# chrhansk/sleqp

Hardware: AMD Instinct MI355X
Metric: KKT factor+solve/sec (numeric refactor + 1 solve with device-controlled refinement, inputs resident in HBM) (higher is better)
Workload: dtype f64; 1 GPU; banded_n1e5_m5e4; n=100000, m=50000, N=150000, nnz_J=1000000, nnz_tril_K=1100000, nnz_L=11646539, nnz_L_stored=12226637, supernodes=569, etree_levels=10, refine_steps=1, hip_graphs=5, solves_per_factor=1, parallelism=single

## Files before the change

sleqp_amd/csrc/abi_options.inc:

```
enum OptionEffect {
  FX_NONE,
  FX_GRAPHS,
  FX_GRAPHS_IF_CHANGED,
  FX_PLANS,
  FX_PLANS_IF_CHANGED,
};
struct OptionRow {
  const char* name;
  const char* env;
  OptionEffect effect;
  int (*set)(hipfact_handle* h, double v);
  const char* doc;
};
#define OPT_STORE(field, conv)                 \
  [](hipfact_handle* h, double v) -> int {     \
    const auto x = (conv);                     \
    const bool changed = h->field != x;        \
    h->field = x;                              \
    return changed;                            \
  }
static const OptionRow kOptions[] = {
    {"refine_steps", "HIPFACT_REFINE", FX_GRAPHS,
     [](hipfact_handle* h, double v) -> int {
       h->refine_steps = std::max(0, (int)v);
// ... 146 lines not shown
    {"profile", nullptr, FX_NONE,
     [](hipfact_handle* h, double v) -> int {
       if (h->prof.on) prof_collect(h);
       if (v < 0)
         for (int c = 0; c < PC_COUNT; ++c) h->prof.ms[c] = 0, h->prof.max_ms[c] = 0, h->prof.cnt[c] = 0;
       h->prof.tagged.clear();
       h->prof.on = v > 0;
       return 1;
     },
     "event-time every kernel class; value < 0 resets the counters"},
    {"ordering", nullptr, FX_PLANS, OPT_STORE(prm.ordering, (int)v),
     "0 nested dissection + AMD leaves (default), 1 AMD on the whole graph, 2 natural"},
    {"max_children", nullptr, FX_PLANS, OPT_STORE(prm.max_children, (int)v),
     "relaxed amalgamation keeps fronts at this many children (default 4 = what the pull extend-add takes in one block)"},
    {"force_generic", nullptr, FX_PLANS, OPT_STORE(prm.force_generic, v != 0.0),
     "1: no saddle-point structure detection, static 1 x 1 pivots on K as given (symmetric positive definite input: the PSD shim)"},
    {"dense_mode", nullptr, FX_PLANS, OPT_STORE(prm.dense_mode, std::min(2, std::max(0, (int)v))),
     "1: late elimination inside the tree (default), 2: low-rank correction, 0: off"},
    {nullptr, "HIPFACT_DATAFLOW_RETRY", FX_NONE, OPT_STORE(df_retry_every, std::max(0, (int)v)), nullptr},
    {nullptr, "HIPFACT_CHECK_LAUNCHES", FX_NONE, OPT_STORE(check_launches, v != 0.0), nullptr},
    {nullptr, "HIPFACT_SOL_SPLIT", FX_NONE, OPT_STORE(sol_split, v != 0.0), nullptr},
    {nullptr, "HIPFACT_IDX64", FX_NONE, OPT_STORE(idx64, v != 0.0), nullptr},
    {nullptr, "HIPFACT_XCD_CLASSES", FX_NONE, OPT_STORE(xcd_classes, std::max(1, std::min(XCD_CLASSES_MAX, (int)v))), nullptr},
};
#undef OPT_STORE

static void options_from_environment(hipfact_handle* h) {
  for (const OptionRow& row : kOptions)
    if (const char* s = row.env ? getenv(row.env) : nullptr) (void)row.set(h, (double)atoi(s));
}

int hipfact_set_option(hipfact_handle* h, const char* name, double value) {
  if (!h || !name) return HIPFACT_EINVAL;
  {
    bool known = false;
    const int rc = multi_set_option(h, name, value, known);
    if (known) return rc;
  }
  {
    bool known = false;
    const int rc = condest_set_option(h, name, value, known);
    if (known) return rc;
  }
  for (const OptionRow& row : kOptions) {
    if (!row.name || strcmp(name, row.name)) continue;
    const int changed = row.set(h, value);
// ... 20 lines not shown
  };
  const Plan& P = h->plan;
  if (!strcmp(name, "perm")) return host_copy(P.perm);
  if (!strcmp(name, "sn_c0")) return host_copy(P.sn_c0);
  if (!strcmp(name, "sn_r")) return host_copy(P.sn_r);
  if (!strcmp(name, "sn_rowptr")) return host_copy(P.sn_rowptr);
  if (!strcmp(name, "sn_rows")) return host_copy(P.sn_rows);
  if (!strcmp(name, "sn_Loff")) return host_copy(P.sn_Loff);
  if (!strcmp(name, "late_cols")) return host_copy(P.late_cols);
  if (!strcmp(name, "sn_level")) return host_copy(P.sn_level);
  if (!strcmp(name, "dense_cols")) return host_copy(P.dense_cols);
  if (!strcmp(name, "cond_history")) return host_copy(h->cond_history);
  const DevBuf* b = nullptr;
  if (!strcmp(name, "L")) b = &h->d_L;
  else if (!strcmp(name, "U")) b = &h->d_U;
  else if (!strcmp(name, "SPf")) b = &h->d_SPf;
  else if (!strcmp(name, "sitems")) b = &h->d_sitems;
  else if (!strcmp(name, "y")) b = &h->d_y;
  else if (!strcmp(name, "xhat")) b = &h->d_xhat;
  else if (!strcmp(name, "ysol")) b = &h->d_ysol;
  else if (!strcmp(name, "uvec")) b = &h->d_uvec;
  else if (!strcmp(name, "dscale")) b = &h->d_dscale;
  else if (!strcmp(name, "Kval")) b = &h->d_Kval;
  else if (!strcmp(name, "mY")) b = &h->d_mY;
  if (!strcmp(name, "cond_d")) {
    const size_t N = (size_t)h->N_ext, off = (2 * COND_T + 3) * N * sizeof(double);
    if (!h->d_cblk.p || bytes > N * sizeof(double)) {
      h->error = "hipfact_debug_copy: unknown buffer or size";
      return HIPFACT_EINVAL;
    }
    HCHECK(h, hipStreamSynchronize(h->stream));
    HCHECK(h, hipMemcpy(out, h->d_cblk.as<char>() + off, bytes, hipMemcpyDeviceToHost));
    return HIPFACT_OK;
  }
  if (!b || !b->p || bytes > b->bytes) {
    h->error = "hipfact_debug_copy: unknown buffer or size";
    return HIPFACT_EINVAL;
  }
  HCHECK(h, hipStreamSynchronize(h->stream));
  HCHECK(h, hipMemcpy(out, b->p, bytes, hipMemcpyDeviceToHost));
  return HIPFACT_OK;
}

int hipfact_debug_place_rows(int m, const int* Ar_ptr, long long fill_bytes, int classes, long long* bounds, int* classes_out,
                             int* grid_out, int* blocks) {
  if (m < 0 || (m > 0 && !Ar_ptr) || fill_bytes < 0 || classes < 1 || classes > XCD_CLASSES_MAX || !bounds || !classes_out ||
// ... 182 lines not shown
  INFO("multi_passes", h->multi_passes) INFO("multi_single_cols", h->multi_single_cols) INFO("multi_failed_col", h->multi_failed_col)
  INFO("multi_sliced_fronts", h->mitems_for < 0 ? 0 : h->n_mcut) INFO("multi_slice_items", h->mitems_for < 0 ? 0 : h->n_mslices) INFO("multi_slice_rows", h->multi_slice_rows)
  INFO("cond_estimates", h->cond_estimates) INFO("cond_blocks", h->cond_blocks) INFO("cond_last", h->cond_last) INFO("condition_estimate", h->condition_estimate)
  INFO("extra_solves", h->extra_solves) INFO("extra_passes", h->extra_passes) INFO("extra_last_status", h->extra_last_status)
  INFO("extra_multi_solves", h->extra_multi_solves) INFO("extra_multi_cols", h->extra_multi_cols) INFO("extra_multi_passes", h->extra_multi_passes)
  INFO("num_solve", h->num_solve) INFO("num_refined", h->solve_cad.num_refined) INFO("refine_adaptive", h->refine_adaptive)
  INFO("num_passes", h->solve_cad.num_passes) INFO("last_omega", h->last_ctl.omega) INFO("last_iters", h->last_ctl.iters)
  INFO("last_status", h->last_ctl.status) INFO("last_tol", h->last_ctl.tol) INFO("kappa_est", h->last_ctl.kappa)
  INFO("refine_inline", h->factor_cad.refine_inline) INFO("refine_tol", h->refine_tol) INFO("equilibrate", h->equilibrate)
  INFO("factor_top_level", h->ftop_level) INFO("factor_top_count", h->ftop_count) INFO("solve_timeouts", h->h_info.p ? h->h_info.as<int>()[INFO_TIMEOUT] : 0)
  INFO("top_level", 1 << 30)
  INFO("use_graph", h->use_graph) INFO("num_graphs", h->graphs.size()) INFO("max_r", P.max_r) INFO("max_w", P.max_w) INFO("refine_steps", h->refine_steps)
  INFO("schur_flops_max_level", h->schur_flops_max)
  INFO("chain_pairs", h->n_pairs)
  INFO("xupd_fused", h->xupd_fused ? 1 : 0)
  INFO("rhs_in_tree", h->last_rhs_in_tree) INFO("xupd_in_tree", h->last_xupd_in_tree) INFO("xupd_blocks_launched", h->last_xupd_blocks)
  INFO("solve_sliced_fronts", h->n_sliced) INFO("solve_resorted_levels", h->n_resorted) INFO("tree_solve", tree_solve(h))
  INFO("refine_check_every", h->refine_check_every) INFO("refine_check_interval", h->solve_cad.check_interval_now) INFO("num_checked", h->solve_cad.num_checked)
  INFO("device", h->device) INFO("nnzM", P.Mi.size()) INFO("nnzA", P.Ar_src.size())
  INFO("rows_total", P.sn_rows.size()) INFO("ent_fused", h->ent_fused) INFO("ent_split", h->ent_split)
  INFO("rows_fused", h->rows_fused) INFO("rows_split", h->rows_split)
  INFO("long_row_segments", h->n_rseg) INFO("row_scale_blocks", row_scale_in_sequence(h) ? h->rs_grid : 0)
  INFO("arena_fill_bytes", arena_fill_bytes(P))
  INFO("xcd_classes", h->xcd_classes) INFO("dealt_multi_item_fronts", h->dealt_multi) INFO("long_prod_segments", h->n_lprod)
  INFO("long_col_segments", h->n_cseg) INFO("idx32", h->idx32) INFO("prod_packed", h->prod_packed)
  INFO("active_bounds", h->maps_on ? h->n_bounds : 0)
  INFO("values_in_place",
       h->have_plan && (!h->from_jacobian || (virtual_current(h) && h->vj->identity))) INFO("inactive_rows", h->maps_on ? h->n_inactive : 0)
#undef INFO
  return HIPFACT_EINVAL;
}
```

sleqp_amd/csrc/kernel_types.h:

```cpp
#pragma once
#include <hip/hip_runtime.h>

#include "device_types.h"

namespace hipfact {

constexpr int FB = 256;
constexpr int MV_LONG = 4096;
constexpr int CL = 8;
constexpr int SB = 1024;
constexpr int DOT_BLOCKS = 128;
constexpr int RL = 16;
constexpr int ST = 1024;
constexpr int SPB = 512;
constexpr int ZT = 64;
constexpr int ZC = 32;
constexpr int ZS = 512;
constexpr int CG_BLOCKS = 2048;
constexpr int CG_CHUNK = 8;

constexpr int MR = 16;
constexpr int MB = 1024;

struct RefineCtl {
// ... 53 lines not shown
  double* __restrict__ segpart;
  unsigned int* __restrict__ segcnt;
};
struct RhsIn {
  const int* __restrict__ Ar_ptr;
  const int* __restrict__ Ar_col;
  const double* __restrict__ Ar_val;
  const int* __restrict__ perm;
  SaddleMaps M;
  const double* __restrict__ b;
};
struct XupdIn {
  int n;
  const int* __restrict__ Kp;
  const double* __restrict__ Ksc;
  const int* __restrict__ Kc_y;
  const int* __restrict__ perm;
  SaddleMaps M;
  const double* __restrict__ b;
  double* __restrict__ z;
  int acc;
  int nblocks;
  double* __restrict__ dot_out;
};
struct CgCtl {
  double rg, z_nrm_sq, rel_tol_sq, rad_sq, alpha, beta, tau;
  double ray_min, ray_max;
  int state;
  int stop, apply, it, max_iter, pad;
};
struct LzCtl {
  double tol, rad_sq, gamma0;
  double gam_prev, gam_cur;
  double del_cur;
  double piv, fsub;
  double rho, s_nrm_sq, sp, p_nrm_sq;
  int k;
  int stop;
  int state;
  int kmax;
};

}
```

sleqp_amd/csrc/kernels_saddle.inc:

```




__global__ __launch_bounds__(FB) void k_row_scale(int m, const int* __restrict__ Ar_ptr,
                                                  const int* __restrict__ Ar_col, const int* __restrict__ Ar_src,
                                                  const double* __restrict__ Kval, const int* __restrict__ vmap,
                                                  const int* __restrict__ dmask, const int* __restrict__ perm,
                                                  int late_my, int enable, double* __restrict__ dscale,
                                                  double* __restrict__ Ar_val, double* __restrict__ Ar_full,
                                                  double* __restrict__ Ksc, double* __restrict__ Kprod,
                                                  double* __restrict__ Kcopy, long long nnzK,
                                                  double2* __restrict__ zero,
                                                  long long nzero, int* __restrict__ info, int nrseg,
                                                  const LongSeg* __restrict__ rseg, DecideIn D, int decide,
                                                  ClassBounds RB) {
  const int nbw = gridDim.x, bid = blockIdx.x;
  if (bid == 0) {
    if (decide && D.ctl->pending) dev_refine_decide(D, 1);
    __syncthreads();
    if (threadIdx.x < INFO_BYTES / 4) info[threadIdx.x] = 0;
  }
  if (Kcopy)
    for (long long i = bid * (long long)FB + threadIdx.x; i < nnzK; i += (long long)nbw * FB) Kcopy[i] = Kval[i];
  const int sub = threadIdx.x % RL;
// ... 150 lines not shown
                                                   const int* __restrict__ perm, SaddleMaps M,
                                                   const double* __restrict__ b, double* __restrict__ t,
                                                   const int* __restrict__ skip) {
  if (skip && *skip) return;
  const RhsIn R{Ar_ptr, Ar_col, Ar_val, perm, M, b};
  const int sub = threadIdx.x % RL;
  const int rpb = FB / RL;
  for (int k = blockIdx.x * rpb + threadIdx.x / RL; k < m; k += gridDim.x * rpb) {
    const double s = rhs_row(R, k, sub);
    if (sub == 0 && R.Ar_ptr[k + 1] - R.Ar_ptr[k] <= LONG_ROW) t[k] = s;
  }
  if (M.nrseg > 0) {
    __shared__ double lsum[FB / 64];
    rhs_long_rows<FB>(R, blockIdx.x, gridDim.x, t, lsum);
  }
}

template <bool ACC>
__global__ __launch_bounds__(FB) void k_x_saddle(int n, int m, const int* __restrict__ Kp,
                                                 const double* __restrict__ Ksc, const int* __restrict__ Kc_y,
                                                 const int* __restrict__ perm, SaddleMaps M,
                                                 const double* __restrict__ yp, const double* __restrict__ b,
                                                 double* __restrict__ z, const int* __restrict__ skip,
                                                 int* __restrict__ epoch) {
  if (skip && *skip) return;
  if (epoch && blockIdx.x == 0 && threadIdx.x == 0) *epoch += 1;
  const int sub = threadIdx.x % CL;
  const int cpb = FB / CL;
  for (int j = blockIdx.x * cpb + threadIdx.x / CL; j < n; j += gridDim.x * cpb) {
    double s = 0.0;
    const int e1 = Kp[j + 1];
    if (e1 - Kp[j] - 1 > LONG_COL) continue;
    for (int e = Kp[j] + 1 + sub; e < e1; e += CL) s += Ksc[e] * yp[Kc_y[e]];
#pragma unroll
    for (int o = CL / 2; o > 0; o >>= 1) s += __shfl_down(s, o, CL);
    if (sub == 0) (void)x_col_write(M, j, s, b, z, ACC ? 1 : 0);
  }
  if (M.ncseg > 0) {
    __shared__ double lsum[FB / 64];
    (void)x_long_cols<false, FB>(M, blockIdx.x, gridDim.x, Kp, Ksc, Kc_y, yp, b, z, ACC ? 1 : 0, nullptr, lsum);
  }
  for (int k = blockIdx.x * FB + threadIdx.x; k < m; k += gridDim.x * FB) {
    const int i = ext_row(M, perm[k]);
    if (i >= 0) {
      const double v = yp[k] * M.dscale[k];
      if (ACC)
        z[i] += v;
      else
        z[i] = v;
    }
  }
}


__device__ __forceinline__ void resid_col_tail(const SaddleMaps& M, int j, double s, const double* __restrict__ b,
                                               const double* __restrict__ z, double* __restrict__ res, double& mr,
                                               double& mb, double& mz) {
  const double bj = b[j], zj = z[j];
  const int v = M.vmap ? M.vmap[j] : -1;
// ... 14 lines not shown
}
__device__ __forceinline__ void resid_row_tail(const SaddleMaps& M, int k, const int* __restrict__ perm, double s,
                                               const double* __restrict__ b, const double* __restrict__ z,
                                               double* __restrict__ res, double& mr, double& mb, double& mz) {
  const int i = ext_row(M, perm[k]);
  if (i >= 0) {
    const double d = M.dscale[k];
    const double bi = b[i] * d;
    const double ri = bi - s;
    res[i] = ri / d;
    mr = nanmax(mr, fabs(ri));
    mb = fmax(mb, fabs(bi));
    mz = fmax(mz, fabs(z[i] / d));
  }
}

__global__ __launch_bounds__(FB) void k_residual_saddle(int n, int m, const int* __restrict__ Kp,
                                                        const int* __restrict__ Ki, const double* __restrict__ Kval,
                                                        const int* __restrict__ Ar_ptr, const int* __restrict__ Ar_col,
                                                        const double* __restrict__ Ar_val,
                                                        const int* __restrict__ perm, SaddleMaps M,
                                                        const double* __restrict__ b, const double* __restrict__ z,
                                                        double* __restrict__ res, const RefineCtl* __restrict__ ctl,
                                                        double* __restrict__ partials, int first, int* __restrict__ defer) {
  if (ctl && !first && ctl->done) return;
  double mr = 0.0, mb = 0.0, mz = 0.0;
  __shared__ double lsum[FB / 64];
  const int nbx = (int)gridDim.x >> 1;
  if ((int)blockIdx.x < nbx) {
    const int sub = threadIdx.x % CL;
    const int cpb = FB / CL;
    const int iters = (n + nbx * cpb - 1) / (nbx * cpb);
    for (int it = 0; it < iters; ++it) {
      const int j = (it * nbx + blockIdx.x) * cpb + threadIdx.x / CL;
      double s = 0.0;
      bool mine = j < n;
      if (mine) {
        const int e1 = Kp[j + 1];
        if (e1 - Kp[j] - 1 > LONG_COL)
          mine = false;
        else
          for (int e = Kp[j] + sub; e < e1; e += CL) {
            const int i = Ki[e];
            const int zi = i < n ? i : ext_row(M, i - n);
            if (zi >= 0) s += Kval[e] * z[zi];
          }
      }
#pragma unroll
      for (int o = CL / 2; o > 0; o >>= 1) s += __shfl_down(s, o, CL);
      if (sub == 0 && mine) resid_col_tail(M, j, s, b, z, res, mr, mb, mz);
    }
    for (int q = blockIdx.x; q < M.ncseg; q += nbx) {
      const LongSeg sg = M.cseg[q];
      const int j = sg.id;
      double s = 0.0;
// ... 78 lines not shown
```

sleqp_amd/csrc/kernels_solve.hip:

```cpp
#include <hip/hip_runtime.h>

#include "device_types.h"
#include "kernel_types.h"

namespace hipfact {
#include "kernels_common.inc"
#include "kernels_residual_common.inc"
#include "kernels_solve_level.inc"
#include "kernels_solve_multi.inc"
#include "kernels_solve_tree.inc"
#include "kernels_saddle.inc"
#include "kernels_vector.inc"
}

#define DENSE_COLS_KERNELS
#include "dense_cols.inc"
#undef DENSE_COLS_KERNELS
#define KRYLOV_DEVICE_KERNELS
#include "krylov_device.inc"
#undef KRYLOV_DEVICE_KERNELS
#define KRYLOV_LSQR_KERNELS
#include "krylov_lsqr.inc"
#undef KRYLOV_LSQR_KERNELS

// ... 17 lines not shown
INST_CGH(64)
#undef INST_CGH
#define INST_LZ(L)                                                                                                  \
  template __global__ void k_lz_spmv_dot<L>(int, const LzCtl*, const int*, const int*, const double*, const int*,   \
                                            const int*, const double*, const double*, double*, double*);
INST_LZ(1)
INST_LZ(4)
INST_LZ(16)
INST_LZ(64)
#undef INST_LZ
#define INST_LSQR(L)                                                                                                  \
  template __global__ void k_lsqr_forward<L>(int, int, const int*, const int*, const double*, const double*,         \
                                             const int*, const int*, const double*, const double*, double, double,   \
                                             double*, double*);                                                      \
  template __global__ void k_lsqr_adjoint<L>(int, int, const int*, const int*, const double*, const double*,         \
                                             const int*, const int*, const double*, const double*, const double*,    \
                                             int, double*, double*);
INST_LSQR(1)
INST_LSQR(4)
INST_LSQR(16)
INST_LSQR(64)
#undef INST_LSQR
template __global__ void k_x_saddle<true>(int, int, const int*, const double*, const int*, const int*, SaddleMaps,
                                          const double*, const double*, double*, const int*, int*);
template __global__ void k_x_saddle<false>(int, int, const int*, const double*, const int*, const int*, SaddleMaps,
                                           const double*, const double*, double*, const int*, int*);
}
```

sleqp_amd/csrc/kernels_solve_tree.inc:

```

__device__ __forceinline__ void dev_refine_decide(const DecideIn& D, int first) {
  RefineCtl* __restrict__ ctl = D.ctl;
  RefineCtl* __restrict__ hctl = D.hctl;
  __shared__ double sh[3][16];
  const int tid = threadIdx.x, nthr = blockDim.x;
  double r = 0.0, bb = 0.0, zz = 0.0;
  for (int q = tid; q < D.nblk; q += nthr) {
    r = nanmax(r, D.partials[3 * q]);
    bb = nanmax(bb, D.partials[3 * q + 1]);
    zz = nanmax(zz, D.partials[3 * q + 2]);
  }
#pragma unroll
  for (int o = 32; o > 0; o >>= 1) {
    r = nanmax(r, __shfl_down(r, o, 64));
    bb = nanmax(bb, __shfl_down(bb, o, 64));
    zz = nanmax(zz, __shfl_down(zz, o, 64));
  }
  if ((tid & 63) == 0) {
    sh[0][tid >> 6] = r;
    sh[1][tid >> 6] = bb;
    sh[2][tid >> 6] = zz;
  }
  __syncthreads();
  if (tid == 0) {
// ... 512 lines not shown
                                              double* __restrict__ z, int acc) {
  const int v = M.vmap ? M.vmap[j] : -1;
  const double bj = b[j];
  if (v >= 0) {
    const double beta = b[v];
    const double mult = (bj - beta) - s;
    if (acc) {
      z[j] += beta;
      z[v] += mult;
    } else {
      z[j] = beta;
      z[v] = mult;
    }
    return bj * beta;
  }
  if (acc) {
    z[j] += bj - s;
    return 0.0;
  }
  const double zj = bj - s;
  z[j] = zj;
  return bj * zj;
}
template <bool POLL, int NT>
__device__ __forceinline__ double x_long_cols(const SaddleMaps& M, int bid, int nb, const int* __restrict__ Kp,
                                              const double* __restrict__ Ksc, const int* __restrict__ Kc_y,
                                              const double* __restrict__ ys, const double* __restrict__ b,
                                              double* __restrict__ z, int acc, int* __restrict__ info, double* lds) {
  double dsum = 0.0;
  for (int q = bid; q < M.ncseg; q += nb) {
    const LongSeg sg = M.cseg[q];
    double s = 0.0;
    for (int e = sg.begin + (int)threadIdx.x; e < sg.end; e += NT)
      s += Ksc[e] * (POLL ? poll_f64(ys + Kc_y[e], info) : ys[Kc_y[e]]);
    s = block_sum_fixed<NT>(s, lds);
    double tot;
    if (threadIdx.x == 0 && seg_arrive(s, sg.poff, sg.idx, sg.nseg, M.segpart, M.segcnt + sg.uid, tot))
      dsum += x_col_write(M, sg.id, tot, b, z, acc);
  }
  return dsum;
}
__device__ __forceinline__ void dev_x_update(const XupdIn& X, int xb, const double* __restrict__ ys, int m,
                                             int* __restrict__ info, double* lds) {
  constexpr int XL = 8, XE = 2, XP = 4;
  const int sub = threadIdx.x % XL;
  const int cpb = ST / XL;
  const int stride = X.nblocks * cpb;
  const SaddleMaps& M = X.M;
  const unsigned long long* __restrict__ yb = reinterpret_cast<const unsigned long long*>(ys);
  const int k0 = xb * ST + threadIdx.x, kstride = X.nblocks * ST;
  int yi = -1;
  double ysc = 0.0, dsum = 0.0;
  if (k0 < m) {
    yi = ext_row(M, X.perm[k0]);
    ysc = M.dscale[k0];
  }
  for (int jb = xb * cpb + threadIdx.x / XL; jb < X.n; jb += XP * stride) {
    double val[XP][XE];
    int idx[XP][XE], enext[XP], eend[XP];
    bool colok[XP];
#pragma unroll
    for (int p = 0; p < XP; ++p) {
      const int j = jb + p * stride;
      bool ok = j < X.n;
      int e0 = ok ? X.Kp[j] + 1 + sub : 0, e1 = ok ? X.Kp[j + 1] : 0;
      if (e1 - (e0 - sub) > LONG_COL) e1 = e0 = 0, ok = false;
      colok[p] = ok;
#pragma unroll
      for (int t = 0; t < XE; ++t) {
        const int e = e0 + XL * t;
        val[p][t] = (e < e1) ? X.Ksc[e] : 0.0;
        idx[p][t] = (e < e1) ? X.Kc_y[e] : -1;
      }
      enext[p] = e0 + XL * XE;
      eend[p] = e1;
    }
    unsigned long long bits[XP][XE];
#pragma unroll
    for (int p = 0; p < XP; ++p)
#pragma unroll
      for (int t = 0; t < XE; ++t)
        bits[p][t] = (idx[p][t] >= 0) ? __hip_atomic_load(yb + idx[p][t], __ATOMIC_RELAXED, __HIP_MEMORY_SCOPE_AGENT) : 0ull;
#pragma unroll
    for (int p = 0; p < XP; ++p) {
      const int j = jb + p * stride;
      double s = 0.0;
#pragma unroll
      for (int t = 0; t < XE; ++t)
        if (idx[p][t] >= 0) {
          const double yv = (bits[p][t] == SOLVE_SENT) ? poll_f64(ys + idx[p][t], info) : __longlong_as_double((long long)bits[p][t]);
          s += val[p][t] * yv;
        }
      for (int e = enext[p]; e < eend[p]; e += XL) s += X.Ksc[e] * poll_f64(ys + X.Kc_y[e], info);
#pragma unroll
      for (int o = XL / 2; o > 0; o >>= 1) s += __shfl_down(s, o, XL);
      if (sub == 0 && colok[p]) dsum += x_col_write(M, j, s, X.b, X.z, X.acc);
    }
  }
  if (M.ncseg > 0) {
    const double dl = x_long_cols<true, ST>(M, xb, X.nblocks, X.Kp, X.Ksc, X.Kc_y, ys, X.b, X.z, X.acc, info, lds);
    if (threadIdx.x == 0) dsum += dl;
    __syncthreads();
  }
  if (X.dot_out) {
    dsum = wave_sum(dsum);
    if ((threadIdx.x & 63) == 0) lds[threadIdx.x >> 6] = dsum;
    __syncthreads();
    if (threadIdx.x == 0) {
      double a = 0.0;
      for (int q = 0; q < ST / 64; ++q) a += lds[q];
      X.dot_out[xb] = a;
    }
  }
  for (int k = k0; k < m; k += kstride) {
    const int i = (k == k0) ? yi : ext_row(M, X.perm[k]);
    if (i >= 0) {
      const double v = poll_f64(ys + k, info) * ((k == k0) ? ysc : M.dscale[k]);
      if (X.acc)
        X.z[i] += v;
// ... 68 lines not shown
```

sleqp_amd/csrc/runtime_extra.inc:

```

struct ExtraRule {
  int nblk = 1, cap = 1;
  int k = 0;
  int applied = 0;
  int status = -1;
  double rho = 0.0, ferr = INFINITY, dz_rel = INFINITY;
  double dn_prev[2] = {0.0, 0.0};
};
static inline double extra_rel(double dn, double zn) { return dn == 0.0 ? 0.0 : dn / zn; }
static bool extra_rule_step(ExtraRule& R, const double* dn, const double* zn) {
  const double eps = std::ldexp(1.0, -53);
  ++R.k;
  bool finite = true;
  for (int q = 0; q < R.nblk; ++q) finite = finite && std::isfinite(dn[q]) && std::isfinite(zn[q]);
  if (!finite) {
    R.status = HIPFACT_EXTRA_NONFINITE;
    R.ferr = R.dz_rel = INFINITY;
    return false;
  }
  double ratio = 0.0;
  if (R.k >= 2) {
    for (int q = 0; q < R.nblk; ++q)
      if (R.dn_prev[q] > 0.0) ratio = std::max(ratio, dn[q] / R.dn_prev[q]);
    R.rho = std::max(R.rho, ratio);
// ... 15 lines not shown
    R.status = HIPFACT_EXTRA_PASS_LIMIT;
  return true;
}

static void residual_dd_async(hipfact_handle* h, const double* b, const double* z, double* res, double* partials) {
  const Plan& P = h->plan;
  if (P.saddle) {
    LAUNCH(PC_RESID, k_residual_saddle_dd, dim3(resid_blocks(P)), dim3(FB), 0, P.n, P.m, h->d_Kp.as<int>(),
           h->d_Ki.as<int>(), h->d_Kval.as<double>(), h->d_Ar_ptr.as<int>(), h->d_Ar_col.as<int>(),
           (masked_rows(h) ? h->d_Ar_full : h->d_Ar_val).as<double>(), h->d_perm.as<int>(), saddle_maps(h), b, z, res,
           partials);
  } else {
    LAUNCH(PC_RESID, k_residual_sym_dd, dim3(resid_blocks(P)), dim3(FB), 0, P.N, h->d_Kp.as<int>(), h->d_Ki.as<int>(),
           h->d_Kval.as<double>(), h->d_Tp.as<int>(), h->d_Ti.as<int>(), h->d_Tsrc.as<int>(), b, z, res, partials);
  }
}

static void residual_fp64_async(hipfact_handle* h, const double* b, const double* z, double* res) {
  const Plan& P = h->plan;
  if (P.saddle) {
    LAUNCH(PC_RESID, k_residual_saddle, dim3(resid_blocks(P)), dim3(FB), 0, P.n, P.m, h->d_Kp.as<int>(),
           h->d_Ki.as<int>(), h->d_Kval.as<double>(), h->d_Ar_ptr.as<int>(), h->d_Ar_col.as<int>(),
           (masked_rows(h) ? h->d_Ar_full : h->d_Ar_val).as<double>(), h->d_perm.as<int>(), saddle_maps(h), b, z, res,
           (const RefineCtl*)nullptr, (double*)nullptr, 1, (int*)nullptr);
  } else {
    LAUNCH(PC_RESID, k_residual_sym, dim3(resid_blocks(P)), dim3(FB), 0, P.N, h->d_Kp.as<int>(), h->d_Ki.as<int>(),
           h->d_Kval.as<double>(), h->d_Tp.as<int>(), h->d_Ti.as<int>(), h->d_Tsrc.as<int>(), b, z, res,
           (const RefineCtl*)nullptr, (double*)nullptr, 1, (int*)nullptr);
  }
}

static const int g_maxabs_cap = 256;

static int extra_workspace(hipfact_handle* h) {
  const size_t N = (size_t)h->N_ext;
  hipError_t e = h->d_xvec.ensure(std::max<size_t>(4 * N * sizeof(double), 16));
  if (e == hipSuccess) e = h->d_xctl.ensure(sizeof(RefineCtl));
  if (e == hipSuccess) e = h->d_xnorms.ensure((size_t)3 * g_resid_cap * sizeof(double));
  if (e == hipSuccess) e = h->d_xpart.ensure((size_t)4 * g_maxabs_cap * sizeof(double));
  if (e == hipSuccess && !h->h_xout.p) {
    e = h->h_xout.ensure(4 * sizeof(double) + sizeof(RefineCtl));
    if (e == hipSuccess) e = hipHostGetDevicePointer(&h->h_xout_dev, h->h_xout.p, 0);
  }
  if (e != hipSuccess) {
    (void)hipGetLastError();
    h->d_xvec.release();
    h->error = std::string("hipfact_solve_device_extra: workspace: ") + hipGetErrorString(e);
// ... 106 lines not shown
```

sleqp_amd/csrc/runtime_queue.inc:

```
struct TurnState {
  std::mutex mu;
  hipEvent_t last = nullptr;
  hipfact_handle* owner = nullptr;
  std::atomic<int> live{0};
};
static TurnState g_turn[16];
static hipfact_handle* g_trace_handles[8] = {nullptr};
struct Turn {
  hipfact_handle* h;
  bool counted = false, held = false;
  explicit Turn(hipfact_handle* h_) : h(h_) {
    if (h->capturing) return;
    counted = true;
    if (h->turn_depth++ > 0) return;
    TurnState& T = g_turn[h->device & 15];
    static const bool off = getenv("HIPFACT_NO_TURNS") != nullptr;
    if (off || T.live.load(std::memory_order_acquire) <= 1 || !h->ev_turn) return;
    T.mu.lock();
    held = true;
    if (T.last && T.owner != h) {
      (void)hipStreamWaitEvent(h->stream, T.last, 0);
      h->turn_waits++;
    }
  }
// ... 21 lines not shown
      break;
    }
}
static void turn_leave(hipfact_handle* h) {
  TurnState& T = g_turn[h->device & 15];
  std::lock_guard<std::mutex> g(T.mu);
  T.live.fetch_sub(1, std::memory_order_acq_rel);
  for (auto& g : g_trace_handles)
    if (g == h) g = nullptr;
  if (T.owner == h) {
    T.owner = nullptr;
    T.last = nullptr;
  }
}

static DecideIn decide_in(hipfact_handle* h, int col = -1);
static inline bool diag_inactive_needed(const hipfact_handle* h) {
  const Plan& P = h->plan;
  return P.saddle && P.m > 0 && ((h->maps_on && h->n_inactive > 0) || P.n_late > 0);
}
static inline bool row_scale_in_sequence(const hipfact_handle* h) {
  const Plan& P = h->plan;
  return P.saddle && P.n > 0 && P.m > 0;
}
static inline bool dataflow_factor(const hipfact_handle* h) { return h->debug_phases == 15 && !h->no_dataflow; }
static inline bool tree_solve(const hipfact_handle* h) { return h->fused_solve && !h->no_dataflow; }
static inline bool tree_delivers_verdict(const hipfact_handle* h) { return tree_solve(h) && h->plan.m > 0 && h->plan.saddle; }
static inline bool graph_route(const hipfact_handle* h) { return h->use_graph && !h->prof.on && h->debug_phases == 15; }
static inline const int* cmap_or_null(const hipfact_handle* h) { return (h->maps_on || h->plan.n_late > 0) ? h->d_cmap.as<int>() : nullptr; }
static inline bool masked_rows(const hipfact_handle* h) { return h->nd > 0 || h->plan.n_late > 0; }
static inline size_t arena_fill_bytes(const Plan& P) {
  return (size_t)P.L_size * sizeof(double) + (size_t)4 * P.nsuper * sizeof(int);
}
static inline int row_scale_grid(long long m, size_t fill_bytes) {
  const long long nz16 = (long long)((fill_bytes + 15) / 16);
  const int for_fill = (int)std::min<long long>(2048, std::max<long long>(1, nz16 / (FB * 8)));
  return std::max(nblocks(m * 16), for_fill);
}
static int place_rows(int m, const int* Ar_ptr, size_t fill_bytes, int classes, ClassBounds& cb) {
  return place_ranges((long long)m, FB / RL, Ar_ptr, LONG_ROW, classes, row_scale_grid(m, fill_bytes), (long long)((fill_bytes + 15) / 16), cb);
}
static void place_front_end(hipfact_handle* h) {
  const Plan& P = h->plan;
  h->rs_grid = place_rows(P.m, P.Ar_ptr.data(), arena_fill_bytes(P), h->xcd_classes, h->rs_place);
}
template <bool CH>
// ... 350 lines not shown
           h->d_info.as<int>(), skip, rhs ? *rhs : RhsIn{},
           decide_in(h), h->d_spart.as<double>(), X);
    return;
  }
  for (int l = 0; l < P.nlevels; ++l) {
    const LevelInfo& li = h->levels[l];
    LAUNCH(PC_FWD, k_fwd_level, dim3(li.count), dim3(SB), li.lds_fwd, h->d_sn.as<SnDesc>(),
           h->d_level_sn.as<int>() + li.begin, h->d_L.as<double>(), h->d_rel.as<int>(), h->d_child.as<int>(),
           h->d_y.as<double>(), h->d_uvec.as<double>(), skip);
  }
  for (int l = P.nlevels - 1; l >= 0; --l) {
    const LevelInfo& li = h->levels[l];
    LAUNCH(PC_BWD, k_bwd_level, dim3(li.count), dim3(SB), li.lds_bwd, h->d_sn.as<SnDesc>(),
           h->d_level_sn.as<int>() + li.begin, h->d_L.as<double>(), h->d_rows.as<int>(), h->d_y.as<double>(), skip);
  }
}

static void launch_rhs_saddle(hipfact_handle* h, const SaddleMaps& M, const double* b, const int* skip, double* y = nullptr) {
  const Plan& P = h->plan;
  LAUNCH(PC_RHS, k_rhs_saddle, dim3(nblocks((long long)P.m * 16)), dim3(FB), 0, P.m, h->d_Ar_ptr.as<int>(),
         h->d_Ar_col.as<int>(), h->d_Ar_val.as<double>(), h->d_perm.as<int>(), M, b, y ? y : h->d_y.as<double>(), skip);
}
static void launch_x_saddle(hipfact_handle* h, const SaddleMaps& M, const double* b, double* z, bool acc, const int* skip,
                            int* epoch, const double* y = nullptr) {
  const Plan& P = h->plan;
  auto go = [&](auto ACC) {
    LAUNCH(PC_XUPD, k_x_saddle<decltype(ACC)::value>, dim3(nblocks((long long)P.n * 8)), dim3(FB), 0, P.n, P.m, h->d_Kp.as<int>(),
           h->d_Ksc.as<double>(), h->d_Kc_y.as<int>(), h->d_perm.as<int>(), M, y ? y : h->d_y.as<double>(), b, z, skip, epoch);
  };
  acc ? go(std::true_type()) : go(std::false_type());
}

static void launch_rhs_perm(hipfact_handle* h, const double* b, const int* skip, double* y = nullptr) {
  const Plan& P = h->plan;
  LAUNCH(PC_PERM, k_gather_skip, dim3(nblocks(P.m)), dim3(FB), 0, (long long)P.m, h->d_perm.as<int>(), b,
         y ? y : h->d_y.as<double>(), skip);
}
static void launch_x_perm(hipfact_handle* h, double* z, bool acc, const int* skip, int* epoch, const double* y = nullptr) {
  const Plan& P = h->plan;
  if (!y) y = h->d_y.as<double>();
  if (acc)
    LAUNCH(PC_PERM, k_scatter_acc, dim3(nblocks(P.m)), dim3(FB), 0, (long long)P.m, h->d_perm.as<int>(), y, z, skip, epoch);
  else
    LAUNCH(PC_PERM, k_scatter, dim3(nblocks(P.m)), dim3(FB), 0, (long long)P.m, h->d_perm.as<int>(), y, z, epoch);
}

static void solve_once_async(hipfact_handle* h, const double* b, double* z, bool acc, const int* skip, bool raw = false) {
  Turn turn(h);
  const Plan& P = h->plan;
  if (h->N_ext == 0) return;
  if (h->nd > 0 && !raw) {
    double* const dot_req = h->x_dot_out;
    h->x_dot_out = nullptr;
    solve_once_async(h, b, h->d_dtmp.as<double>(), false, skip, true);
    h->x_dot_out = dot_req;
    dense_correct_async(h, z, acc, skip);
    return;
  }
  const bool tree = tree_solve(h);
  int* epoch = (tree && P.m > 0) ? h->d_epoch.as<int>() : nullptr;
  h->last_rhs_in_tree = h->last_xupd_in_tree = h->last_xupd_blocks = 0;
  if (P.saddle) {
    const SaddleMaps M = saddle_maps(h);
    const bool rhs_in_tree = tree && h->rhs_fused && h->n_lrows == 0;
    const bool whole = tree && h->rhs_fused && h->xupd_fused && P.n > 0 && P.m > 0;
    if (P.m > 0) {
      if (!rhs_in_tree) launch_rhs_saddle(h, M, b, skip);
      const RhsIn R{rhs_in_tree ? h->d_Ar_ptr.as<int>() : nullptr, h->d_Ar_col.as<int>(), h->d_Ar_val.as<double>(), h->d_perm.as<int>(), M, b};
      XupdIn X;
      memset(&X, 0, sizeof(X));
      if (whole) {
        X.n = P.n;
        X.Kp = h->d_Kp.as<int>();
        X.Ksc = h->d_Ksc.as<double>();
        X.Kc_y = h->d_Kc_y.as<int>();
        X.perm = h->d_perm.as<int>();
        X.M = M;
        X.b = b;
        X.z = z;
        X.acc = acc ? 1 : 0;
        X.nblocks = std::max(1, std::min(h->xupd_blocks, (P.n + (ST / 8) - 1) / (ST / 8)));
        if (h->x_dot_out && !acc) {
          X.dot_out = h->x_dot_out;
          h->x_dot_blocks = X.nblocks;
        }
      }
      h->last_rhs_in_tree = rhs_in_tree;
      h->last_xupd_in_tree = whole;
      h->last_xupd_blocks = X.nblocks;
      solve_m_async(h, skip, (rhs_in_tree || whole) ? &R : nullptr, whole ? &X : nullptr);
    }
    if (!whole) launch_x_saddle(h, M, b, z, acc, skip, epoch);
  } else {
    launch_rhs_perm(h, b, skip);
    solve_m_async(h, skip);
    launch_x_perm(h, z, acc, skip, epoch);
  }
}

static const int g_resid_cap = 2048;
static inline int resid_blocks(const Plan& P) {
  return P.saddle ? std::max(2, nblocks((long long)P.N * 8, g_resid_cap) & ~1) : nblocks(P.N, g_resid_cap);
}

static DecideIn decide_in(hipfact_handle* h, int col) {
  const bool own = col >= 0;
  const size_t j = own ? (size_t)col : 0;
  return DecideIn{(own ? h->d_mctl : h->d_ctl).as<RefineCtl>() + j, static_cast<RefineCtl*>(own ? h->h_mctl_dev : h->h_ctl_dev) + j,
                  (own ? h->d_mnorms : h->d_norms).as<double>() + j * 3 * g_resid_cap, resid_blocks(h->plan),
                  h->refine_adaptive ? h->refine_tol : -1.0, minmax_ptr(h)};
}

static void residual_async(hipfact_handle* h, const double* b, const double* z, double* res, bool first,
                           bool defer = false, int col = -1) {
  const Plan& P = h->plan;
  const DecideIn D = decide_in(h, col);
  RefineCtl* ctl = D.ctl;
  double* norms = const_cast<double*>(D.partials);
  int* dflag = defer ? &ctl->pending : nullptr;
  if (P.saddle) {
    LAUNCH(PC_RESID, k_residual_saddle, dim3(resid_blocks(P)), dim3(FB), 0, P.n, P.m, h->d_Kp.as<int>(),
           h->d_Ki.as<int>(), h->d_Kval.as<double>(), h->d_Ar_ptr.as<int>(), h->d_Ar_col.as<int>(),
           (masked_rows(h) ? h->d_Ar_full : h->d_Ar_val).as<double>(), h->d_perm.as<int>(), saddle_maps(h), b, z, res, ctl,
           norms,
           first ? 1 : 0, dflag);
  } else {
    LAUNCH(PC_RESID, k_residual_sym, dim3(resid_blocks(P)), dim3(FB), 0, P.N, h->d_Kp.as<int>(), h->d_Ki.as<int>(),
           h->d_Kval.as<double>(), h->d_Tp.as<int>(), h->d_Ti.as<int>(), h->d_Tsrc.as<int>(), b, z, res, ctl,
           norms, first ? 1 : 0, dflag);
  }
  if (!defer) LAUNCH(PC_RESID, k_refine_decide, dim3(1), dim3(FB), 0, D, first ? 1 : 0, 0);
}

static void flush_decide(hipfact_handle* h) {
  if (!cadence(h).verdict_outstanding()) return;
  hipLaunchKernelGGL(k_refine_decide, dim3(1), dim3(FB), 0, h->stream, decide_in(h), 1, 1);
  cadence(h).verdict_flushed();
}

static void drop_graphs(hipfact_handle* h) {
  h->graphs.clear();
  for (auto& st : h->cache) st->graphs.clear();
}
static void drop_solve_graphs(hipfact_handle* h) {
  std::vector<GraphEntry> keep;
  for (auto& g : h->graphs.v) {
    if (g.kind == 0)
      keep.push_back(g);
// ... 45 lines not shown
  const hipError_t ei = hipGraphInstantiate(&exec, graph, nullptr, nullptr, 0);
  (void)hipGraphDestroy(graph);
  if (ei != hipSuccess || !exec) {
    (void)hipGetLastError();
    h->use_graph = false;
    return direct();
  }
  if (h->graphs.size() >= 16) drop_graphs(h);
  h->graphs.push_back({kind, b, z, passes, exec});
  return launch(exec);
}

static int correct_enqueue(hipfact_handle* h, const double* bb, double* z, int passes) {
  const int* skip = &h->d_ctl.as<RefineCtl>()->done;
  for (int it = 0; it < passes; ++it) {
    solve_once_async(h, h->d_res.as<double>(), z, true, skip);
    residual_async(h, bb, z, h->d_res.as<double>(), false);
  }
  HCHECK(h, hipGetLastError());
  return HIPFACT_OK;
}

static inline int top_block_key(const hipfact_handle* h) { return h->tb_valid ? 1000 : 0; }

static int solve_enqueue(hipfact_handle* h, const double* b, double* z, const hipfact::SolveDecision& d) {
  const double* bb = b;
  if (h->refine_steps > 0 && b == z) {
    HCHECK(h, hipMemcpyAsync(h->d_rhs.p, b, (size_t)h->N_ext * sizeof(double), hipMemcpyDeviceToDevice, h->stream));
    bb = h->d_rhs.as<double>();
  }
  solve_once_async(h, bb, z, false, nullptr);
  if (h->refine_steps > 0 && !d.unchecked) {
    residual_async(h, bb, z, h->d_res.as<double>(), true, d.defer);
    return correct_enqueue(h, bb, z, d.passes);
  }
  HCHECK(h, hipGetLastError());
  return HIPFACT_OK;
}

static int top_block_build(hipfact_handle* h) {
  const int nT = h->tb_nT;
  hipStream_t st = h->stream;
  HCHECK(h, hipMemsetAsync(h->d_tb_xd.p, 0, (size_t)nT * nT * sizeof(double), st));
  HCHECK(h, hipMemsetAsync(h->d_tb_xhat.p, 0xFF, (size_t)4 * nT * sizeof(double), st));
  HCHECK(h, hipMemsetAsync(h->d_tb_gathered.p, 0, 16, st));
  hipLaunchKernelGGL(k_top_inverse, dim3(h->tb_nchunks), dim3(ST), 0, st, h->d_tb_chunks.as<TopChunk>(),
                     h->d_tb_fronts.as<TopFront>(), h->d_sitems.as<SolveItem>(), h->d_SPf.as<double>(), h->d_rows.as<int>(),
                     h->d_tb_tl.as<int>(), h->d_tb_xd.as<double>(), nT);
  TopBlockIn TB;
  memset(&TB, 0, sizeof(TB));
  TB.nT = nT;
  TB.ntf = h->tb_ntf;
  TB.items = h->d_tb_items.as<TopBlockItem>();
  {
    HCHECK(h, h->d_tb_zd.ensure((size_t)nT * nT * sizeof(double)));
    const int nt = (nT + ZT - 1) / ZT;
// ... 19 lines not shown
  h->note('T', 0);
  return HIPFACT_OK;
}

static int top_block_touch(hipfact_handle* h) {
  const int after = (h->solves_prev_factor >= h->top_block_breakeven) ? h->top_block_after
                                                                       : std::max(h->top_block_after, h->top_block_breakeven);
  if (!h->tb_valid && h->tb_nT > 0 && h->top_block_after > 0 && h->solves_this_factor >= after &&
      tree_solve(h) && !h->prof.on && h->debug_phases == 15)
    return top_block_build(h);
  return HIPFACT_OK;
}

static int solve_async(hipfact_handle* h, const double* b, double* z, bool all_checked = false) {
  h->sol_prefetched = false;
  if (h->N_ext == 0) return HIPFACT_OK;
  ++h->solves_this_factor;
  if (int rc = top_block_touch(h)) return rc;
  hipfact::Cadence cad = cadence(h);
  const hipfact::CadenceKnobs knobs = cadence_knobs(h);
  const hipfact::SolveDecision d = cad.solve_decision(knobs, tree_delivers_verdict(h),
                                                      cad.wants_peek(knobs) ? ctl_peek_pinned(h) : hipfact::CtlPeek{-1, 0, 0, 0, 0.0, 0.0}, all_checked);
  if (d.flush_first) flush_decide(h);
  const int key = d.key + top_block_key(h);
  h->note(d.unchecked ? 'U' : 'S', key);
  const int rc = d.unchecked ? solve_enqueue(h, b, z, d) : run_cached(h, 1, b, z, [&] { return solve_enqueue(h, b, z, d); }, key);
  if (rc) return rc;
  cad.solve_queued(knobs, d);
  h->num_solve++;
  h->solved = true;
  h->last_b = (b == z) ? h->d_rhs.as<double>() : b;
  h->last_z = z;
  return HIPFACT_OK;
}

static bool vtable_can_retry(const hipfact_handle* h);
static int vtable_retry_exact(hipfact_handle* h);
static bool static_pivot_applies(const hipfact_handle* h);
static int static_pivot_retry(hipfact_handle* h, int rc);

enum class Verdict { accepted, stalled, out_of_range };
static Verdict refine_verdict(const hipfact_handle* h, const RefineCtl& c) {
  if (!h->refine_adaptive || c.status == 2) return Verdict::accepted;
  if (c.omega > h->fail_omega) return Verdict::stalled;
  if (h->reg_delta > 0.0 && c.rnorm > h->fail_omega * c.bnorm) return Verdict::out_of_range;
  return Verdict::accepted;
}
static void set_verdict_error(hipfact_handle* h, Verdict v, const RefineCtl& c, int col = -1) {
  char of_col[32] = "", subject[48] = "the right-hand side", buf[260];
// ... 278 lines not shown
```

sleqp_amd/csrc/runtime_types.inc:

```
namespace hipfact {

struct DevBuf {
  void* p = nullptr;
  size_t bytes = 0;
  DevBuf() = default;
  DevBuf(const DevBuf&) = delete;
  DevBuf& operator=(const DevBuf&) = delete;
  DevBuf(DevBuf&& o) noexcept : p(o.p), bytes(o.bytes) {
    o.p = nullptr;
    o.bytes = 0;
  }
  DevBuf& operator=(DevBuf&& o) noexcept {
    if (this != &o) {
      release();
      p = o.p;
      bytes = o.bytes;
      o.p = nullptr;
      o.bytes = 0;
    }
    return *this;
  }
  ~DevBuf() { release(); }
  void release() {
    if (p) (void)hipFree(p);
// ... 275 lines not shown
  long dense_probes = 0;
  bool decide_rides = false;
  const double* vals_ride = nullptr;
  bool use_graph = true;
  bool no_dataflow = false;
  int fake_timeouts = 0;
  long dataflow_fallbacks = 0;
  int df_retry_every = 256;
  long df_retry_at = -1;
  long dataflow_rearmed = 0;
  int debug_phases = 15;
  int solve_whole_max = 48;
  bool factor_hint_peek = true;
  int top_block_breakeven = 48;
  bool chain_pairs = true;
  int n_pairs = 0;
  long long pair_extra = 0;
  double schur_flops_max = 0.0;
  bool check_launches = false, launch_reported = false;
  double* x_dot_out = nullptr;
  int x_dot_blocks = 0;
  int xupd_blocks = 256;
  bool solve_sorted = true;
  int xcd_classes = 8;
  int factor_top_max = 160;
  int factor_top_levels = 1 << 20;
  int factor_top_max_u = 1024;
  int factor_top_fine = 12;
  int top_block_after = 2;
  int top_block_max = 2048;
  long tb_builds = 0;
  bool factor_top_head = true;
  int factor_top_fused = 30;
  int factor_top_fused32 = 12;
  int factor_top_fused_u = 256;
  int factor_top_post = 64;
  int panel_small_below = 0;
  int pull_max_children = 4;
  long cache_hits = 0, analyses = 0, num_factor = 0;
  int info_host[INFO_WORDS] = {0, 0, 0, 0};
  Prof prof;
  DevBuf d_info, d_norms, d_ctl;
  PinBuf h_ctl;
  void* h_ctl_dev = nullptr;
  PinBuf h_stage, h_info;
  DevBuf d_sp_idx, d_sp_val;
// ... 128 lines not shown
```

Baseline: 1502 factor+solve/s.

## Compute x-block residual inside the x-update kernel instead of residual pass

The x-update step of the saddle-point solve (both the standalone kernel and the in-tree fused path) now also computes the residual rows for the x block. It reuses the products it already loaded and adds the diagonal term from Kval. The residual kernel then only handles the remaining rows and the norm reductions, with fewer blocks (grid shifted by from_x, default 3). This removes a second sparse matvec over the Jacobian columns. In exchange the x-update does extra work per column, and the feature is gated by plan conditions and a new graph cache key.

```diff
diff --git a/sleqp_amd/csrc/abi_options.inc b/sleqp_amd/csrc/abi_options.inc
--- a/sleqp_amd/csrc/abi_options.inc
+++ b/sleqp_amd/csrc/abi_options.inc
@@ -192,6 +192,7 @@
     {nullptr, "HIPFACT_SOL_SPLIT", FX_NONE, OPT_STORE(sol_split, v != 0.0), nullptr},
     {nullptr, "HIPFACT_IDX64", FX_NONE, OPT_STORE(idx64, v != 0.0), nullptr},
     {nullptr, "HIPFACT_XCD_CLASSES", FX_NONE, OPT_STORE(xcd_classes, std::max(1, std::min(XCD_CLASSES_MAX, (int)v))), nullptr},
+    {nullptr, "HIPFACT_RESID_FROM_X", FX_NONE, OPT_STORE(resid_from_x, std::max(0, std::min(3, (int)v))), nullptr},
 };
 #undef OPT_STORE
 
@@ -258,6 +259,8 @@
   else if (!strcmp(name, "uvec")) b = &h->d_uvec;
   else if (!strcmp(name, "dscale")) b = &h->d_dscale;
   else if (!strcmp(name, "Kval")) b = &h->d_Kval;
+  else if (!strcmp(name, "res")) b = &h->d_res;
+  else if (!strcmp(name, "norms")) b = &h->d_norms;
   else if (!strcmp(name, "mY")) b = &h->d_mY;
   if (!strcmp(name, "cond_d")) {
     const size_t N = (size_t)h->N_ext, off = (2 * COND_T + 3) * N * sizeof(double);
@@ -486,6 +489,7 @@
   INFO("rows_fused", h->rows_fused) INFO("rows_split", h->rows_split)
   INFO("long_row_segments", h->n_rseg) INFO("row_scale_blocks", row_scale_in_sequence(h) ? h->rs_grid : 0)
   INFO("arena_fill_bytes", arena_fill_bytes(P))
+  INFO("resid_blocks", resid_blocks(P)) INFO("resid_from_x", resid_from_x(h)) INFO("resid_queued_from_x", h->resid_queued_from_x) INFO("resid_queued_full", h->resid_queued_full)
   INFO("xcd_classes", h->xcd_classes) INFO("dealt_multi_item_fronts", h->dealt_multi) INFO("long_prod_segments", h->n_lprod)
   INFO("long_col_segments", h->n_cseg) INFO("idx32", h->idx32) INFO("prod_packed", h->prod_packed)
   INFO("active_bounds", h->maps_on ? h->n_bounds : 0)
diff --git a/sleqp_amd/csrc/kernel_types.h b/sleqp_amd/csrc/kernel_types.h
--- a/sleqp_amd/csrc/kernel_types.h
+++ b/sleqp_amd/csrc/kernel_types.h
@@ -99,6 +99,8 @@
   int acc;
   int nblocks;
   double* __restrict__ dot_out;
+  const double* __restrict__ Kval;
+  double* __restrict__ res;
 };
 struct CgCtl {
   double rg, z_nrm_sq, rel_tol_sq, rad_sq, alpha, beta, tau;
diff --git a/sleqp_amd/csrc/kernels_saddle.inc b/sleqp_amd/csrc/kernels_saddle.inc
--- a/sleqp_amd/csrc/kernels_saddle.inc
+++ b/sleqp_amd/csrc/kernels_saddle.inc
@@ -196,19 +196,26 @@
                                                  const int* __restrict__ perm, SaddleMaps M,
                                                  const double* __restrict__ yp, const double* __restrict__ b,
                                                  double* __restrict__ z, const int* __restrict__ skip,
-                                                 int* __restrict__ epoch) {
+                                                 int* __restrict__ epoch, const double* __restrict__ Kval,
+                                                 double* __restrict__ res) {
   if (skip && *skip) return;
   if (epoch && blockIdx.x == 0 && threadIdx.x == 0) *epoch += 1;
   const int sub = threadIdx.x % CL;
   const int cpb = FB / CL;
   for (int j = blockIdx.x * cpb + threadIdx.x / CL; j < n; j += gridDim.x * cpb) {
     double s = 0.0;
-    const int e1 = Kp[j + 1];
-    if (e1 - Kp[j] - 1 > LONG_COL) continue;
-    for (int e = Kp[j] + 1 + sub; e < e1; e += CL) s += Ksc[e] * yp[Kc_y[e]];
+    const int e0 = Kp[j] + 1 + sub, e1 = Kp[j + 1];
+    if (e1 - (e0 - sub) > LONG_COL) continue;
+    for (int e = e0; e < e1; e += CL) s += Ksc[e] * yp[Kc_y[e]];
+    const double part = s;
 #pragma unroll
     for (int o = CL / 2; o > 0; o >>= 1) s += __shfl_down(s, o, CL);
     if (sub == 0) (void)x_col_write(M, j, s, b, z, ACC ? 1 : 0);
+    if (!ACC && res)
+      x_col_resid(M, j, sub, true, part, s, b, sub == CL - 1 ? Kval[e0 - CL] : 0.0, res, [&](double r) {
+        for (int e = e0; e < e1; e += CL) r += Ksc[e] * yp[Kc_y[e]];
+        return r;
+      });
   }
   if (M.ncseg > 0) {
     __shared__ double lsum[FB / 64];
@@ -269,15 +276,33 @@
                                                         const int* __restrict__ perm, SaddleMaps M,
                                                         const double* __restrict__ b, const double* __restrict__ z,
                                                         double* __restrict__ res, const RefineCtl* __restrict__ ctl,
-                                                        double* __restrict__ partials, int first, int* __restrict__ defer) {
+                                                        double* __restrict__ partials, int first, int* __restrict__ defer,
+                                                        int from_x) {
   if (ctl && !first && ctl->done) return;
   double mr = 0.0, mb = 0.0, mz = 0.0;
   __shared__ double lsum[FB / 64];
-  const int nbx = (int)gridDim.x >> 1;
+  const int nbx = from_x > 0 ? max(1, (int)gridDim.x >> from_x) : (int)gridDim.x >> 1;
   if ((int)blockIdx.x < nbx) {
     const int sub = threadIdx.x % CL;
     const int cpb = FB / CL;
-    const int iters = (n + nbx * cpb - 1) / (nbx * cpb);
+    const int iters = from_x > 0 ? 0 : (n + nbx * cpb - 1) / (nbx * cpb);
+    if (from_x > 0)
+      for (int j = blockIdx.x * FB + threadIdx.x; j < n; j += nbx * FB) {
+        if (M.ncseg > 0 && Kp[j + 1] - Kp[j] - 1 > LONG_COL) continue;
+        const double bj = b[j], zj = z[j], rj = res[j];
+        const int v = M.vmap ? M.vmap[j] : -1;
+        if (v >= 0) {
+          const double zv = z[v], bv = b[v];
+          const double rv = bv - zj;
+          res[v] = rv;
+          mr = nanmax(mr, fabs(rv));
+          mb = fmax(mb, fabs(bv));
+          mz = fmax(mz, fabs(zv));
+        }
+        mr = nanmax(mr, fabs(rj));
+        mb = fmax(mb, fabs(bj));
+        mz = fmax(mz, fabs(zj));
+      }
     for (int it = 0; it < iters; ++it) {
       const int j = (it * nbx + blockIdx.x) * cpb + threadIdx.x / CL;
       double s = 0.0;
diff --git a/sleqp_amd/csrc/kernels_solve.hip b/sleqp_amd/csrc/kernels_solve.hip
--- a/sleqp_amd/csrc/kernels_solve.hip
+++ b/sleqp_amd/csrc/kernels_solve.hip
@@ -63,7 +63,7 @@
 INST_LSQR(64)
 #undef INST_LSQR
 template __global__ void k_x_saddle<true>(int, int, const int*, const double*, const int*, const int*, SaddleMaps,
-                                          const double*, const double*, double*, const int*, int*);
+                                          const double*, const double*, double*, const int*, int*, const double*, double*);
 template __global__ void k_x_saddle<false>(int, int, const int*, const double*, const int*, const int*, SaddleMaps,
-                                           const double*, const double*, double*, const int*, int*);
+                                           const double*, const double*, double*, const int*, int*, const double*, double*);
 }
diff --git a/sleqp_amd/csrc/kernels_solve_tree.inc b/sleqp_amd/csrc/kernels_solve_tree.inc
--- a/sleqp_amd/csrc/kernels_solve_tree.inc
+++ b/sleqp_amd/csrc/kernels_solve_tree.inc
@@ -558,6 +558,35 @@
   z[j] = zj;
   return bj * zj;
 }
+template <class Resum>
+__device__ __forceinline__ void x_col_resid(const SaddleMaps& M, int j, int sub, bool ok, double part, double tot,
+                                            const double* __restrict__ b, double diag, double* __restrict__ res,
+                                            Resum resum) {
+  const bool last = ok && sub == CL - 1;
+  tot = __shfl(tot, 0, CL);
+  double s = part, bj = 0.0, mult = 0.0;
+  int v = -1;
+  if (last) {
+    bj = b[j];
+    v = M.vmap ? M.vmap[j] : -1;
+    double zj;
+    if (v >= 0) {
+      const double beta = b[v];
+      zj = beta;
+      mult = (bj - beta) - tot;
+    } else
+      zj = bj - tot;
+    s = 0.0;
+    s += diag * zj;
+    s = resum(s);
+  }
+#pragma unroll
+  for (int o = CL / 2; o > 0; o >>= 1) s += __shfl(s, (sub + o) & (CL - 1), CL);
+  if (last) {
+    if (v >= 0) s += mult;
+    res[j] = bj - s;
+  }
+}
 template <bool POLL, int NT>
 __device__ __forceinline__ double x_long_cols(const SaddleMaps& M, int bid, int nb, const int* __restrict__ Kp,
                                               const double* __restrict__ Ksc, const int* __restrict__ Kc_y,
@@ -592,7 +621,7 @@
     ysc = M.dscale[k0];
   }
   for (int jb = xb * cpb + threadIdx.x / XL; jb < X.n; jb += XP * stride) {
-    double val[XP][XE];
+    double val[XP][XE], dg[XP];
     int idx[XP][XE], enext[XP], eend[XP];
     bool colok[XP];
 #pragma unroll
@@ -610,6 +639,7 @@
       }
       enext[p] = e0 + XL * XE;
       eend[p] = e1;
+      dg[p] = (X.res && ok && sub == XL - 1) ? X.Kval[e0 - XL] : 0.0;
     }
     unsigned long long bits[XP][XE];
 #pragma unroll
@@ -620,17 +650,26 @@
 #pragma unroll
     for (int p = 0; p < XP; ++p) {
       const int j = jb + p * stride;
-      double s = 0.0;
+      double s = 0.0, yv[XE];
 #pragma unroll
       for (int t = 0; t < XE; ++t)
         if (idx[p][t] >= 0) {
-          const double yv = (bits[p][t] == SOLVE_SENT) ? poll_f64(ys + idx[p][t], info) : __longlong_as_double((long long)bits[p][t]);
-          s += val[p][t] * yv;
+          yv[t] = (bits[p][t] == SOLVE_SENT) ? poll_f64(ys + idx[p][t], info) : __longlong_as_double((long long)bits[p][t]);
+          s += val[p][t] * yv[t];
         }
       for (int e = enext[p]; e < eend[p]; e += XL) s += X.Ksc[e] * poll_f64(ys + X.Kc_y[e], info);
+      const double part = s;
 #pragma unroll
       for (int o = XL / 2; o > 0; o >>= 1) s += __shfl_down(s, o, XL);
       if (sub == 0 && colok[p]) dsum += x_col_write(M, j, s, X.b, X.z, X.acc);
+      if (X.res)
+        x_col_resid(M, j, sub, colok[p], part, s, X.b, dg[p], X.res, [&](double r) {
+#pragma unroll
+          for (int t = 0; t < XE; ++t)
+            if (idx[p][t] >= 0) r += val[p][t] * yv[t];
+          for (int e = enext[p]; e < eend[p]; e += XL) r += X.Ksc[e] * poll_f64(ys + X.Kc_y[e], info);
+          return r;
+        });
     }
   }
   if (M.ncseg > 0) {
diff --git a/sleqp_amd/csrc/runtime_extra.inc b/sleqp_amd/csrc/runtime_extra.inc
--- a/sleqp_amd/csrc/runtime_extra.inc
+++ b/sleqp_amd/csrc/runtime_extra.inc
@@ -61,7 +61,7 @@
     LAUNCH(PC_RESID, k_residual_saddle, dim3(resid_blocks(P)), dim3(FB), 0, P.n, P.m, h->d_Kp.as<int>(),
            h->d_Ki.as<int>(), h->d_Kval.as<double>(), h->d_Ar_ptr.as<int>(), h->d_Ar_col.as<int>(),
            (masked_rows(h) ? h->d_Ar_full : h->d_Ar_val).as<double>(), h->d_perm.as<int>(), saddle_maps(h), b, z, res,
-           (const RefineCtl*)nullptr, (double*)nullptr, 1, (int*)nullptr);
+           (const RefineCtl*)nullptr, (double*)nullptr, 1, (int*)nullptr, 0);
   } else {
     LAUNCH(PC_RESID, k_residual_sym, dim3(resid_blocks(P)), dim3(FB), 0, P.N, h->d_Kp.as<int>(), h->d_Ki.as<int>(),
            h->d_Kval.as<double>(), h->d_Tp.as<int>(), h->d_Ti.as<int>(), h->d_Tsrc.as<int>(), b, z, res,
diff --git a/sleqp_amd/csrc/runtime_queue.inc b/sleqp_amd/csrc/runtime_queue.inc
--- a/sleqp_amd/csrc/runtime_queue.inc
+++ b/sleqp_amd/csrc/runtime_queue.inc
@@ -67,6 +67,10 @@
 static inline bool row_scale_in_sequence(const hipfact_handle* h) {
   const Plan& P = h->plan;
   return P.saddle && P.n > 0 && P.m > 0;
+}
+static inline int resid_from_x(const hipfact_handle* h) {
+  const Plan& P = h->plan;
+  return (P.saddle && P.n > 0 && P.m > 0 && h->nd == 0 && P.n_late == 0 && h->refine_steps > 0) ? h->resid_from_x : 0;
 }
 static inline bool dataflow_factor(const hipfact_handle* h) { return h->debug_phases == 15 && !h->no_dataflow; }
 static inline bool tree_solve(const hipfact_handle* h) { return h->fused_solve && !h->no_dataflow; }
@@ -463,11 +467,12 @@
          h->d_Ar_col.as<int>(), h->d_Ar_val.as<double>(), h->d_perm.as<int>(), M, b, y ? y : h->d_y.as<double>(), skip);
 }
 static void launch_x_saddle(hipfact_handle* h, const SaddleMaps& M, const double* b, double* z, bool acc, const int* skip,
-                            int* epoch, const double* y = nullptr) {
+                            int* epoch, const double* y = nullptr, double* res = nullptr) {
   const Plan& P = h->plan;
   auto go = [&](auto ACC) {
     LAUNCH(PC_XUPD, k_x_saddle<decltype(ACC)::value>, dim3(nblocks((long long)P.n * 8)), dim3(FB), 0, P.n, P.m, h->d_Kp.as<int>(),
-           h->d_Ksc.as<double>(), h->d_Kc_y.as<int>(), h->d_perm.as<int>(), M, y ? y : h->d_y.as<double>(), b, z, skip, epoch);
+           h->d_Ksc.as<double>(), h->d_Kc_y.as<int>(), h->d_perm.as<int>(), M, y ? y : h->d_y.as<double>(), b, z, skip, epoch,
+           h->d_Kval.as<double>(), acc ? nullptr : res);
   };
   acc ? go(std::true_type()) : go(std::false_type());
 }
@@ -501,6 +506,7 @@
   const bool tree = tree_solve(h);
   int* epoch = (tree && P.m > 0) ? h->d_epoch.as<int>() : nullptr;
   h->last_rhs_in_tree = h->last_xupd_in_tree = h->last_xupd_blocks = 0;
+  double* const x_res = (acc || raw) ? nullptr : h->x_res_out;
   if (P.saddle) {
     const SaddleMaps M = saddle_maps(h);
     const bool rhs_in_tree = tree && h->rhs_fused && h->n_lrows == 0;
@@ -525,13 +531,15 @@
           X.dot_out = h->x_dot_out;
           h->x_dot_blocks = X.nblocks;
         }
+        X.Kval = h->d_Kval.as<double>();
+        X.res = x_res;
       }
       h->last_rhs_in_tree = rhs_in_tree;
       h->last_xupd_in_tree = whole;
       h->last_xupd_blocks = X.nblocks;
       solve_m_async(h, skip, (rhs_in_tree || whole) ? &R : nullptr, whole ? &X : nullptr);
     }
-    if (!whole) launch_x_saddle(h, M, b, z, acc, skip, epoch);
+    if (!whole) launch_x_saddle(h, M, b, z, acc, skip, epoch, nullptr, x_res);
   } else {
     launch_rhs_perm(h, b, skip);
     solve_m_async(h, skip);
@@ -553,7 +561,7 @@
 }
 
 static void residual_async(hipfact_handle* h, const double* b, const double* z, double* res, bool first,
-                           bool defer = false, int col = -1) {
+                           bool defer = false, int col = -1, int from_x = 0) {
   const Plan& P = h->plan;
   const DecideIn D = decide_in(h, col);
   RefineCtl* ctl = D.ctl;
@@ -564,7 +572,8 @@
            h->d_Ki.as<int>(), h->d_Kval.as<double>(), h->d_Ar_ptr.as<int>(), h->d_Ar_col.as<int>(),
            (masked_rows(h) ? h->d_Ar_full : h->d_Ar_val).as<double>(), h->d_perm.as<int>(), saddle_maps(h), b, z, res, ctl,
            norms,
-           first ? 1 : 0, dflag);
+           first ? 1 : 0, dflag, from_x);
+    ++(from_x > 0 ? h->resid_queued_from_x : h->resid_queued_full);
   } else {
     LAUNCH(PC_RESID, k_residual_sym, dim3(resid_blocks(P)), dim3(FB), 0, P.N, h->d_Kp.as<int>(), h->d_Ki.as<int>(),
            h->d_Kval.as<double>(), h->d_Tp.as<int>(), h->d_Ti.as<int>(), h->d_Tsrc.as<int>(), b, z, res, ctl,
@@ -656,16 +665,21 @@
 }
 
 static inline int top_block_key(const hipfact_handle* h) { return h->tb_valid ? 1000 : 0; }
-
-static int solve_enqueue(hipfact_handle* h, const double* b, double* z, const hipfact::SolveDecision& d) {
+static inline int resid_x_key(int from_x) { return 2000 * from_x; }
+
+static int solve_enqueue(hipfact_handle* h, const double* b, double* z, const hipfact::SolveDecision& d, int from_x) {
   const double* bb = b;
   if (h->refine_steps > 0 && b == z) {
     HCHECK(h, hipMemcpyAsync(h->d_rhs.p, b, (size_t)h->N_ext * sizeof(double), hipMemcpyDeviceToDevice, h->stream));
     bb = h->d_rhs.as<double>();
   }
+  const bool checked = h->refine_steps > 0 && !d.unchecked;
+  if (!checked) from_x = 0;
+  h->x_res_out = from_x > 0 ? h->d_res.as<double>() : nullptr;
   solve_once_async(h, bb, z, false, nullptr);
-  if (h->refine_steps > 0 && !d.unchecked) {
-    residual_async(h, bb, z, h->d_res.as<double>(), true, d.defer);
+  h->x_res_out = nullptr;
+  if (checked) {
+    residual_async(h, bb, z, h->d_res.as<double>(), true, d.defer, -1, from_x);
     return correct_enqueue(h, bb, z, d.passes);
   }
   HCHECK(h, hipGetLastError());
@@ -731,9 +745,10 @@
   const hipfact::SolveDecision d = cad.solve_decision(knobs, tree_delivers_verdict(h),
                                                       cad.wants_peek(knobs) ? ctl_peek_pinned(h) : hipfact::CtlPeek{-1, 0, 0, 0, 0.0, 0.0}, all_checked);
   if (d.flush_first) flush_decide(h);
-  const int key = d.key + top_block_key(h);
+  const int from_x = d.unchecked ? 0 : resid_from_x(h);
+  const int key = d.key + top_block_key(h) + resid_x_key(from_x);
   h->note(d.unchecked ? 'U' : 'S', key);
-  const int rc = d.unchecked ? solve_enqueue(h, b, z, d) : run_cached(h, 1, b, z, [&] { return solve_enqueue(h, b, z, d); }, key);
+  const int rc = d.unchecked ? solve_enqueue(h, b, z, d, 0) : run_cached(h, 1, b, z, [&] { return solve_enqueue(h, b, z, d, from_x); }, key);
   if (rc) return rc;
   cad.solve_queued(knobs, d);
   h->num_solve++;
diff --git a/sleqp_amd/csrc/runtime_types.inc b/sleqp_amd/csrc/runtime_types.inc
--- a/sleqp_amd/csrc/runtime_types.inc
+++ b/sleqp_amd/csrc/runtime_types.inc
@@ -321,6 +321,9 @@
   int x_dot_blocks = 0;
   int xupd_blocks = 256;
   bool solve_sorted = true;
+  int resid_from_x = 3;
+  double* x_res_out = nullptr;
+  long resid_queued_from_x = 0, resid_queued_full = 0;
   int xcd_classes = 8;
   int factor_top_max = 160;
   int factor_top_levels = 1 << 20;
```

Measured after the change: 1519 factor+solve/s, median of 6. 1.1% higher.
